# wienkers/marEx

Hardware: AMD Instinct MI355X
Metric: Mcells*timesteps/s, shifting_baseline + hobday_extreme p95 (validation+anomaly+thresholds+mask) (higher is better)
Workload: dtype f32

## Files before the change

### marex_amd/csrc/marex_tails.hip

```cpp
#include "marex_common.hip.h"
#include "marex_tails.hip.h"

typedef __amdgpu_buffer_rsrc_t tl_rsrc_t;
__device__ __forceinline__ tl_rsrc_t tl_make_rsrc(const void* base) {
    return __builtin_amdgcn_make_buffer_rsrc(const_cast<void*>(base), 0, -1, 0x00020000);
}
__device__ __forceinline__ uint4 tl_load_chunk(tl_rsrc_t r, unsigned voff, unsigned soff) {
    typedef unsigned u4 __attribute__((ext_vector_type(4)));
    const u4 v = __builtin_amdgcn_raw_buffer_load_b128(r, (int)voff, (int)soff, 0);
    return make_uint4(v.x, v.y, v.z, v.w);
}
__device__ __forceinline__ unsigned pk_sub_sat_u16(unsigned a, unsigned b) {
    unsigned r;
    asm("v_pk_sub_u16 %0, %1, %2 clamp" : "=v"(r) : "v"(a), "v"(b));
    return r;
}
__device__ __forceinline__ unsigned pk_add_u16(unsigned a, unsigned b) {
    unsigned r;
    asm("v_pk_add_u16 %0, %1, %2" : "=v"(r) : "v"(a), "v"(b));
    return r;
}
__device__ __forceinline__ unsigned pk_sub_u16(unsigned a, unsigned b) {
    unsigned r;
    asm("v_pk_sub_u16 %0, %1, %2" : "=v"(r) : "v"(a), "v"(b));
// ... 1084 lines not shown
        else if (big && p == 2 && tall)
            MAREX_TT_LAUNCH(2, 30, 1024, 34);
        else if (big && p == 2)
            MAREX_TT_LAUNCH(2, 32, 1024);
        else if (big)
            MAREX_TT_LAUNCH(3, 32, 1024);
        else if (p == 1)
            MAREX_TT_LAUNCH(1, 16, 256);
        else if (p == 2)
            MAREX_TT_LAUNCH(2, 16, 256);
        else
            MAREX_TT_LAUNCH(3, 16, 256);
    }
#undef MAREX_TT_LAUNCH
#undef MAREX_TT_ARGS
    HIP_TRY(ctx, hipGetLastError());
    return 0;
}

template <bool RING>
__global__ void __launch_bounds__(64)
k_thr_pool(const uint4* __restrict__ lists, const unsigned* __restrict__ aux, int NPER, int nch, const float* __restrict__ anom,
           long C, long c0, long c1, int nblk, const int* __restrict__ pool, int K, const float* __restrict__ centres, int nb,
           double q, int wd, float lower_bound, float upper_bound, float* __restrict__ thr, marex_thr_stats* __restrict__ stats,
           unsigned long long* __restrict__ dbg) {
    extern __shared__ uint4 pool_smem[];
    const int lane = (int)threadIdx.x;
    const long cell = c0 + (long)blockIdx.x * 64 + lane;
    const bool valid = cell < c1;
    const int d_begin = (int)blockIdx.y * NDOY / nblk, d_end = ((int)blockIdx.y + 1) * NDOY / nblk;
    const bool land = valid ? !(anom[cell] == anom[cell]) : true;
    if (__builtin_amdgcn_ballot_w64(!land) == 0) {
        if (valid)
            for (int d = d_begin; d < d_end; ++d) thr[(size_t)d * C + cell] = nan_f();
        return;
    }
    int* mem = reinterpret_cast<int*>(pool_smem) + lane;
    for (int m = 0; m < K; ++m) mem[m * 64] = land ? -1 : pool[(size_t)m * C + cell];
    uint4* ring = pool_smem + K * 16 + lane;
    const int pd = wd / 2, per_day = K * NPER, nslot = (wd * per_day + 3) & ~3;
    if (RING)
        for (int k = wd * per_day; k < nslot; ++k) ring[k * 64] = make_uint4(0, 0, 0, 0);
    const unsigned chunk_row = (unsigned)C * 16u;
    const size_t day_stride = (size_t)NPER * nch * (size_t)C;
    auto wrap = [](int d) { return d < 0 ? d + NDOY : (d >= NDOY ? d - NDOY : d); };
    auto cnt_of = [&](int day) {
        int n = 0;
        for (int m = 0; m < K; ++m) {
            const int j = mem[m * 64];
            if (j >= 0) n += (int)(aux[(size_t)day * C + j] & 0x3FFu);
        }
        return n;
    };
    auto global_first = [&](int day, int j, int p) {
        return tl_load_chunk(tl_make_rsrc(lists + (size_t)day * day_stride), (unsigned)j * 16u, (unsigned)(nch * p) * chunk_row);
    };
    auto load_day = [&](int day, int k) {
        if (!RING) return;
        for (int m = 0; m < K; ++m) {
            const int j = mem[m * 64];
            for (int p = 0; p < NPER; ++p) {
                const uint4 ch = j >= 0 ? global_first(day, j, p) : make_uint4(0, 0, 0, 0);
                ring[((k % wd) * per_day + m * NPER + p) * 64] = ch;
            }
        }
    };
    auto first_chunk = [&](int d, int i, int m, int p) {
        if (RING) return ring[(i * per_day + m * NPER + p) * 64];
        const int j = mem[m * 64];
        return j >= 0 ? global_first(wrap(d - pd + i), j, p) : make_uint4(0, 0, 0, 0);
    };
    int tot = 0;
    for (int o = 0; o < wd; ++o) {
        const int day = wrap(d_begin - pd + o);
        load_day(day, o);
        tot += cnt_of(day);
    }
    auto count_first = [&](int d, int b, int& sat) {
        const unsigned lim = ((unsigned)(b + 1) << TAIL_POS_BITS) - 1u, lim_rep = lim | (lim << 16);
        unsigned acc0 = 0, acc1 = 0, accl = 0;
        if (RING) {
            for (int k = 0; k < nslot; k += 4) {
                const uint4 c[4] = {ring[k * 64], ring[(k + 1) * 64], ring[(k + 2) * 64], ring[(k + 3) * 64]};
#pragma unroll
                for (int u = 0; u < 4; ++u) {
                    acc0 += pk_min1_u16(pk_sub_sat_u16(c[u].x, lim_rep)) + pk_min1_u16(pk_sub_sat_u16(c[u].z, lim_rep));
                    acc1 += pk_min1_u16(pk_sub_sat_u16(c[u].y, lim_rep));
                    accl += pk_min1_u16(pk_sub_sat_u16(c[u].w, lim_rep));
                }
            }
        } else
        for (int i = 0; i < wd; ++i)
            for (int m = 0; m < K; ++m)
                for (int p = 0; p < NPER; ++p) {
                    const uint4 c = first_chunk(d, i, m, p);
                    acc0 += pk_min1_u16(pk_sub_sat_u16(c.x, lim_rep)) + pk_min1_u16(pk_sub_sat_u16(c.z, lim_rep));
                    acc1 += pk_min1_u16(pk_sub_sat_u16(c.y, lim_rep));
                    accl += pk_min1_u16(pk_sub_sat_u16(c.w, lim_rep));
                }
        sat = (int)(accl >> 16);
        const unsigned acc = acc0 + acc1 + accl;
        return (int)((acc & 0xFFFFu) + (acc >> 16));
    };
    auto count_behind = [&](int d, int b, bool want) {
        const unsigned lim = ((unsigned)(b + 1) << TAIL_POS_BITS) - 1u, lim_rep = lim | (lim << 16);
        const int s0 = (d - d_begin) % wd;
        int n = 0;
        for (int i = 0; i < wd; ++i) {
            const int o = RING ? (i - s0 + wd) % wd : i;
            const tl_rsrc_t r = tl_make_rsrc(lists + (size_t)wrap(d - pd + o) * day_stride);
            for (int m = 0; m < K; ++m) {
                const int j = mem[m * 64];
                if (j < 0 || !want) continue;
                for (int p = 0; p < NPER; ++p) {
                    const uint4 c = first_chunk(d, i, m, p);
                    if ((c.w >> 16) <= lim) continue;
                    for (int jj = 1; jj < nch; ++jj) n += tl_count_above(tl_load_chunk(r, (unsigned)j * 16u, (unsigned)(nch * p + jj) * chunk_row), lim_rep);
                }
            }
        }
        return n;
    };
    unsigned kmin = 0xFFFFFFFFu, kmax = 0u, nlow = 0u, nhigh = 0u;
    unsigned long long n_exact = 0;
    for (int d = d_begin; d < d_end; ++d) {
        if (d > d_begin) {
            const int din = wrap(d + pd), dout = wrap(d - pd - 1);
            load_day(din, d - d_begin - 1);
            tot += cnt_of(din) - cnt_of(dout);
        }
        unsigned khead = 0, ktail = 0xFFFFu;
        int nlists = 0;
        auto see_head = [&](unsigned first_pair) {
            const unsigned head = first_pair & 0xFFFFu;
            khead = head > khead ? head : khead;
            ktail = (head != 0u && head < ktail) ? head : ktail;
            nlists += head != 0u ? 1 : 0;
        };
        if (RING) {
            for (int k = 0; k < nslot; k += 4) {
                const unsigned h[4] = {ring[k * 64].x, ring[(k + 1) * 64].x, ring[(k + 2) * 64].x, ring[(k + 3) * 64].x};
#pragma unroll
                for (int u = 0; u < 4; ++u) see_head(h[u]);
            }
        } else
        for (int i = 0; i < wd; ++i)
            for (int m = 0; m < K; ++m)
                for (int p = 0; p < NPER; ++p) see_head(first_chunk(d, i, m, p).x);
        float t32 = nan_f();
        if (tot > 0) {
            const double qpos = q * (double)tot;
            int lo = -1, hi = nb - 1, n_lo = tot, n_hi = 0;
            if (khead != 0u && (double)tot > qpos) {
                const int bh = (int)(khead >> TAIL_POS_BITS) - 1;
                hi = bh < hi ? bh : hi;
            }
            bool lo_exact = true;
            if (nlists > 0 && (double)(tot - nlists) <= qpos) {
                const int bt = (int)(ktail >> TAIL_POS_BITS) - 2;
                if (bt > lo && bt < hi) {
                    lo = bt;
                    n_lo = nlists;
                    lo_exact = false;
                }
            }
            while (__builtin_amdgcn_ballot_w64(hi - lo > 1) != 0) {
                const bool go = hi - lo > 1;
                const int mid = go ? (lo + hi) >> 1 : hi;
                int sat;
                int n = count_first(d, mid + 1, sat);
                bool exact = sat == 0;
                bool f = (double)(tot - n) <= qpos;
                const bool undecided = go && !f && !exact;
                if (__builtin_amdgcn_ballot_w64(undecided) != 0) {
                    const int more = count_behind(d, mid + 1, undecided);
                    if (undecided) {
                        n += more;
                        exact = true;
                        f = (double)(tot - n) <= qpos;
                        ++n_exact;
                    }
                }
                if (go) {
                    if (f) {
                        lo = mid;
                        n_lo = n;
                        lo_exact = exact;
                    } else {
                        hi = mid;
                        n_hi = n;
                    }
                }
            }
            const int iu = hi;
            const bool redo = iu > 0 && !lo_exact;
            if (__builtin_amdgcn_ballot_w64(redo) != 0) {
                int sat;
                const int ne = count_first(d, iu, sat) + count_behind(d, iu, redo);
                if (redo) {
                    n_lo = ne;
                    ++n_exact;
                }
            }
            const int il = iu > 0 ? iu - 1 : 0;
            const int cs_iu = tot - n_hi, cs_il = iu > 0 ? tot - n_lo : cs_iu;
            const int diff = cs_iu - cs_il;
            const double frac = diff > 0 ? (qpos - (double)cs_il) / (double)diff : 0.5;
            const float dc = centres[iu] - centres[il];
            const double prod = frac * (double)dc;
            t32 = (float)((double)centres[il] + prod);
            if (iu == 0) t32 = centres[0];
            if (!land) {
                const unsigned key = ordered_key(t32);
                kmin = key < kmin ? key : kmin;
                kmax = key > kmax ? key : kmax;
                if (t32 > upper_bound) ++nhigh;
                if (t32 < lower_bound) ++nlow;
            }
            if (t32 < lower_bound) t32 = lower_bound;
        }
        if (valid) thr[(size_t)d * C + cell] = land ? nan_f() : t32;
    }
    for (int sft = 32; sft > 0; sft >>= 1) {
        const unsigned a = __shfl_down(kmin, sft, 64), b = __shfl_down(kmax, sft, 64);
        kmin = a < kmin ? a : kmin;
        kmax = b > kmax ? b : kmax;
        nlow += __shfl_down(nlow, sft, 64);
        nhigh += __shfl_down(nhigh, sft, 64);
        n_exact += __shfl_down(n_exact, sft, 64);
    }
    if (lane == 0) {
        if (kmin != 0xFFFFFFFFu) atomicMin(&stats->min_key, kmin);
        if (kmax != 0u) atomicMax(&stats->max_key, kmax);
        if (nlow) atomicAdd(&stats->n_too_low, nlow);
        if (nhigh) atomicAdd(&stats->n_too_high, nhigh);
        if (dbg) {
            if (n_exact) atomicAdd(&dbg[1], n_exact);
            atomicAdd(&dbg[0], RING ? 1ull : 0ull);
            atomicAdd(&dbg[2], 1ull);
            atomicAdd(&dbg[3], (unsigned long long)(d_end - d_begin));
        }
    }
}

extern "C" int marex_hobday_thresholds_pool_f32(marex_ctx* ctx, const void* lists, const uint32_t* aux, int list_rows,
                                                const float* anom, int64_t T_out, int64_t C, int max_bucket, const int32_t* pool,
                                                int K, int64_t c0, int64_t c1, const float* centres, int nb, double q, int wd,
                                                float lower_bound, float upper_bound, float* thr_doy_major, marex_thr_stats* stats) {
    if (!ctx) return -1;
    if (!lists || !aux || !anom || !pool || !centres || !thr_doy_major || !stats || T_out <= 0 || C <= 0)
        return fail(ctx, -1, "marex_hobday_thresholds_pool_f32: null pointer or empty shape");
    if (wd < 3 || wd > 365 || (wd & 1) == 0)
        return fail(ctx, -1, "marex_hobday_thresholds_pool_f32: window_days_hobday must be odd and in 3..365");
    if (!(q > 0.0 && q <= 1.0)) return fail(ctx, -1, "marex_hobday_thresholds_pool_f32: q must be in (0, 1]");
    if (K < 1 || K > 13) return fail(ctx, -1, "marex_hobday_thresholds_pool_f32: a pool has 1..13 members (two neighbour rings), not %d", K);
    if (c0 < 0 || c0 >= c1 || c1 > C) return fail(ctx, -1, "marex_hobday_thresholds_pool_f32: need 0 <= c0 < c1 <= C");
    if (nb < 4 || nb > TAIL_MAX_NB || max_bucket < 1 || max_bucket > TAIL_MAX_BUCKET || (int64_t)max_bucket * wd * K > 65535 ||
        C > (1 << 24))
        return fail(ctx, -4, "marex_hobday_thresholds_pool_f32: shape outside the tail kernel (nb <= %d, buckets <= %d rows, "
                             "pooled window <= 65535 samples)", TAIL_MAX_NB, TAIL_MAX_BUCKET);
    HIP_TRY(ctx, hipSetDevice(ctx->device));
    int NPER, nch;
    if (!tails_geometry(max_bucket, list_rows, NPER, nch))
        return fail(ctx, -4, "marex_hobday_thresholds_pool_f32: %d rows per bucket in lists of %d", max_bucket, list_rows);
    {
        std::vector<int32_t> h((size_t)K * (size_t)C);
        HIP_TRY(ctx, hipMemcpyAsync(h.data(), pool, h.size() * sizeof(int32_t), hipMemcpyDeviceToHost, ctx->stream));
        HIP_TRY(ctx, hipStreamSynchronize(ctx->stream));
        for (int64_t c = c0; c < c1; ++c)
            if (h[(size_t)c] != (int32_t)c)
                return fail(ctx, -1, "marex_hobday_thresholds_pool_f32: row 0 of the pool table must be the cell itself (cell %lld lists %d)",
                            (long long)c, (int)h[(size_t)c]);
        for (int m = 1; m < K; ++m)
            for (int64_t c = c0; c < c1; ++c) {
                const int32_t j = h[(size_t)m * (size_t)C + (size_t)c];
                if (j < -1 || j >= C)
                    return fail(ctx, -1, "marex_hobday_thresholds_pool_f32: pool member %d of cell %lld is %d, outside -1..%lld", m,
                                (long long)c, (int)j, (long long)C - 1);
            }
    }
    const int nlist = (wd * K * NPER + 3) & ~3;
    const size_t lds_mem = (size_t)K * 64 * sizeof(int), lds_max = 128 * 1024;
    const size_t lds_ring = lds_mem + (size_t)nlist * 64 * sizeof(uint4);
    const bool use_ring = lds_ring <= lds_max && ctx_opt(ctx, "THR_POOL_RING", 1) != 0;
    const size_t lds = use_ring ? lds_ring : lds_mem;
    const long ncg = (long)((c1 - c0 + 63) / 64);
    int nblk = (int)((32L * 4 * device_cus(ctx) + ncg - 1) / ncg);
    nblk = nblk < 1 ? 1 : (nblk > 12 ? 12 : nblk);
    nblk = ctx_opt(ctx, "THR_POOL_BLOCKS", nblk);
    nblk = nblk < 1 ? 1 : (nblk > NDOY ? NDOY : nblk);
    auto kern = use_ring ? k_thr_pool<true> : k_thr_pool<false>;
    if (lds > 64 * 1024) HIP_TRY(ctx, hipFuncSetAttribute((const void*)kern, hipFuncAttributeMaxDynamicSharedMemorySize, (int)lds));
    LaunchTimer lt(ctx, MAREX_K_THRESHOLDS);
    hipLaunchKernelGGL(kern, dim3((unsigned)ncg, (unsigned)nblk), dim3(64), lds, ctx->stream, reinterpret_cast<const uint4*>(lists),
                       aux, NPER, nch, anom, (long)C, (long)c0, (long)c1, nblk, pool, K, centres, nb, q, wd, lower_bound, upper_bound,
                       thr_doy_major, stats, ctx_debug_counters(ctx));
    HIP_TRY(ctx, hipGetLastError());
    return 0;
}

#ifndef MASK_WAVES
#define MASK_WAVES 5
#endif
template <int NPERT>
__global__ void __launch_bounds__(256, MASK_WAVES)
k_mask_tails(const uint4* __restrict__ lists, const unsigned* __restrict__ aux, int NPER_all, int nch, const float* __restrict__ anom,
             const float* __restrict__ edges, int nb, const float* __restrict__ thr, const int* __restrict__ doy_start,
             const int* __restrict__ doy_rows, const long long* __restrict__ row_off, const long long* __restrict__ row_off_anom,
             long C, long c0, long c1, unsigned char* __restrict__ out, unsigned long long* __restrict__ n_true,
             unsigned long long* __restrict__ dbg) {
    const int nchunk = (int)gridDim.y;
    const int dA = (int)blockIdx.y * NDOY / nchunk, dB = ((int)blockIdx.y + 1) * NDOY / nchunk;
    const long c = (c0 & ~255L) + ((long)blockIdx.x * 256 + threadIdx.x) * 4;
    unsigned cnt_true = 0;
    unsigned long long n_slow = 0;
    if (c >= c0 && c < c1) {
        const float inv_width = (float)(nb - 1) / (edges[nb] - edges[1]);
        for (int d = dA; d < dB; ++d) {
            const int r0 = doy_start[d], nd = doy_start[d + 1] - r0;
            if (nd == 0) continue;
            const float4 th4 = *reinterpret_cast<const float4*>(thr + (size_t)d * C + c);
            const float tv[4] = {th4.x, th4.y, th4.z, th4.w};
            const uint4 ax = *reinterpret_cast<const uint4*>(aux + (size_t)d * C + c);
            const unsigned av[4] = {ax.x, ax.y, ax.z, ax.w};
            unsigned beyond = 0;
            unsigned bits[4][4];
            unsigned lim_ge[4];
            int kt[4];
            bool slow = false, walk[4];
#pragma unroll
            for (int i = 0; i < 4; ++i) {
                bits[i][0] = bits[i][1] = bits[i][2] = bits[i][3] = 0u;
                const bool isnum = tv[i] == tv[i];
                kt[i] = isnum ? digitize_bin(tv[i], edges, nb, inv_width) : nb;
                slow = slow || (isnum && (av[i] & TAIL_AUX_BEYOND) && ((av[i] & TAIL_AUX_MANY) || kt[i] >= nb));
                beyond |= (isnum && (av[i] & TAIL_AUX_BEYOND)) ? 1u : 0u;
                walk[i] = isnum && (av[i] & 0x3FFu) > 0 && kt[i] < nb;
                const unsigned lim = ((unsigned)(kt[i] + 1) << TAIL_POS_BITS) - 1u;
                lim_ge[i] = lim | (lim << 16);
            }
            auto set_prefix = [&](const uint4& q, int n, int i) {
#pragma unroll
                for (int u = 0; u < 8; ++u) {
                    const bool on = n > u;
                    if (u >= 1 && __builtin_amdgcn_ballot_w64(on) == 0) break;
                    if (on) {
                        const int pos = (int)(tl_key(q, u) & (TAIL_MAX_BUCKET - 1));
#pragma unroll
                        for (int wi = 0; wi < 4; ++wi)
                            if ((pos >> 5) == wi) bits[i][wi] |= 1u << (pos & 31);
                    }
                }
            };
            if (__builtin_amdgcn_ballot_w64(!slow) != 0)
            for (int pg = 0; pg < NPER_all; pg += NPERT) {
                const int NPER = (NPER_all - pg) < NPERT ? (NPER_all - pg) : NPERT;
                uint4 ch[NPERT][4];
                const uint4* row0 = lists + (((size_t)d * NPER_all + pg) * nch) * C + c;
#pragma unroll
                for (int p = 0; p < NPERT; ++p)
#pragma unroll
                    for (int i = 0; i < 4; ++i) ch[p][i] = p < NPER ? row0[(size_t)(p * nch) * C + i] : make_uint4(0, 0, 0, 0);
            float cand_val[NPERT][4];
            int cand_pos[NPERT][4];
            unsigned redo = 0;
            {
#pragma unroll
                for (int p = 0; p < NPERT; ++p) {
#pragma unroll
                    for (int i = 0; i < 4; ++i) {
                        cand_pos[p][i] = -1;
                        cand_val[p][i] = 0.f;
                        if (p < NPER && walk[i] && !slow) {
                            const unsigned lgt = lim_ge[i] + (0x10001u << TAIL_POS_BITS);
                            const int n_ge = tl_count_above(ch[p][i], lim_ge[i]);
                            const int n_gt = tl_count_above(ch[p][i], lgt);
                            set_prefix(ch[p][i], n_gt, i);
                            if (n_ge == 8 || n_ge - n_gt > 1) redo |= 1u << (p * 4 + i);
                            if (n_ge - n_gt == 1) {
                                const unsigned w[4] = {ch[p][i].x, ch[p][i].y, ch[p][i].z, ch[p][i].w};
                                unsigned lo = w[0], hi = w[1];
#pragma unroll
                                for (int k = 1; k < 4; ++k)
                                    if ((n_gt >> 1) == k) lo = w[k], hi = k < 3 ? w[k + 1] : 0u;
                                const unsigned key = (n_gt & 1) ? (lo >> 16) : (lo & 0xFFFFu);
                                (void)hi;
                                cand_pos[p][i] = (int)(key & (TAIL_MAX_BUCKET - 1));
                            }
                        }
                    }
                }
#pragma unroll
                for (int p = 0; p < NPERT; ++p)
#pragma unroll
                    for (int i = 0; i < 4; ++i)
                        if (cand_pos[p][i] >= 0)
                            cand_val[p][i] = *reinterpret_cast<const float*>(reinterpret_cast<const char*>(anom) + row_off_anom[r0 + cand_pos[p][i]] + (size_t)(c + i) * 4);
#pragma unroll
                for (int p = 0; p < NPERT; ++p)
#pragma unroll
                    for (int i = 0; i < 4; ++i)
                        if (cand_pos[p][i] >= 0 && cand_val[p][i] >= tv[i]) {
                            const int pos = cand_pos[p][i];
#pragma unroll
                            for (int wi = 0; wi < 4; ++wi)
                                if ((pos >> 5) == wi) bits[i][wi] |= 1u << (pos & 31);
                        }
                if (__builtin_amdgcn_ballot_w64(redo != 0u) != 0) {
#pragma unroll
                    for (int p = 0; p < NPERT; ++p)
#pragma unroll
                        for (int i = 0; i < 4; ++i) {
                            if (__builtin_amdgcn_ballot_w64((redo >> (p * 4 + i)) & 1u) == 0) continue;
                            bool on = (redo >> (p * 4 + i)) & 1u;
                            for (int jj = 0; jj < nch; ++jj) {
                                if (__builtin_amdgcn_ballot_w64(on) == 0) break;
                                const uint4 q = on ? row0[(size_t)(p * nch + jj) * C + i] : make_uint4(0, 0, 0, 0);
#pragma unroll
                                for (int u = 0; u < 8; ++u) {
                                    const unsigned key = tl_key(q, u);
                                    const int bin = (int)(key >> TAIL_POS_BITS) - 1, pos = (int)(key & (TAIL_MAX_BUCKET - 1));
                                    on = on && bin >= kt[i];
                                    if (on) {
                                        bool ext = bin > kt[i];
                                        if (!ext) ext = *reinterpret_cast<const float*>(reinterpret_cast<const char*>(anom) + row_off_anom[r0 + pos] + (size_t)(c + i) * 4) >= tv[i];
                                        if (ext) {
#pragma unroll
                                            for (int wi = 0; wi < 4; ++wi)
                                                if ((pos >> 5) == wi) bits[i][wi] |= 1u << (pos & 31);
                                        }
                                    }
                                }
                            }
                        }
                }
            }
            }
            if (__builtin_amdgcn_ballot_w64(beyond != 0u && !slow) != 0) {
#pragma unroll
                for (int i = 0; i < 4; ++i) {
                    if (!slow && tv[i] == tv[i] && (av[i] & TAIL_AUX_BEYOND)) {
                        const int p1 = (int)((av[i] >> 16) & 0x7Fu), p2 = (int)((av[i] >> 23) & 0x7Fu);
                        const bool two = (av[i] & TAIL_AUX_SECOND) != 0u;
#pragma unroll
                        for (int wi = 0; wi < 4; ++wi) {
                            if ((p1 >> 5) == wi) bits[i][wi] |= 1u << (p1 & 31);
                            if (two && (p2 >> 5) == wi) bits[i][wi] |= 1u << (p2 & 31);
                        }
                    }
                }
            }
            if (slow) {
                ++n_slow;
                for (int r = 0; r < nd; ++r) {
                    const size_t off = (size_t)doy_rows[r0 + r] * C + c;
                    const float4 a = *reinterpret_cast<const float4*>(anom + off);
                    const unsigned m0 = a.x >= tv[0], m1 = a.y >= tv[1], m2 = a.z >= tv[2], m3 = a.w >= tv[3];
                    cnt_true += m0 + m1 + m2 + m3;
                    __builtin_nontemporal_store(m0 | (m1 << 8) | (m2 << 16) | (m3 << 24), reinterpret_cast<unsigned*>(out + off));
                }
            } else {
                unsigned char* obase = out + c;
#pragma unroll
                for (int wi = 0; wi < 4; ++wi) {
                    const unsigned b0 = bits[0][wi], b1 = bits[1][wi], b2 = bits[2][wi], b3 = bits[3][wi];
                    cnt_true += __popc(b0) + __popc(b1) + __popc(b2) + __popc(b3);
                    if (wi * 32 >= nd) break;
#pragma unroll
                    for (int g = 0; g < 4; ++g) {
                        const int rlo = wi * 32 + g * 8;
                        if (rlo >= nd) break;
                        const unsigned q0 = b0 >> (g * 8), q1 = b1 >> (g * 8), q2 = b2 >> (g * 8), q3 = b3 >> (g * 8);
                        const long long* ro = row_off + r0 + rlo;
                        if (rlo + 8 <= nd) {
#pragma unroll
                            for (int rr = 0; rr < 8; ++rr) {
                                const unsigned m = ((q0 >> rr) & 1u) | (((q1 >> rr) & 1u) << 8) | (((q2 >> rr) & 1u) << 16) | (((q3 >> rr) & 1u) << 24);
                                __builtin_nontemporal_store(m, reinterpret_cast<unsigned*>(obase + ro[rr]));
                            }
                        } else {
                            for (int rr = 0; rr < nd - rlo; ++rr) {
                                const unsigned m = ((q0 >> rr) & 1u) | (((q1 >> rr) & 1u) << 8) | (((q2 >> rr) & 1u) << 16) | (((q3 >> rr) & 1u) << 24);
                                __builtin_nontemporal_store(m, reinterpret_cast<unsigned*>(obase + ro[rr]));
                            }
                        }
                    }
                }
            }
        }
    }
    if (n_true) {
        for (int s = 32; s > 0; s >>= 1) cnt_true += __shfl_down(cnt_true, s, 64);
        if ((threadIdx.x & 63) == 0 && cnt_true) atomicAdd(n_true, (unsigned long long)cnt_true);
    }
    if (dbg) {
        for (int s = 32; s > 0; s >>= 1) n_slow += __shfl_down(n_slow, s, 64);
        if ((threadIdx.x & 63) == 0 && n_slow) atomicAdd(&dbg[4], n_slow);
    }
}

extern "C" int marex_mask_ge_doy_tails_f32(marex_ctx* ctx, const void* lists, const uint32_t* aux, int list_rows, int max_bucket,
                                           const float* anom,
                                           const float* edges, int nb, const float* thr_doy_major, const int32_t* doy_start,
                                           const int32_t* doy_rows, int64_t T_out, int64_t C, int64_t c0, int64_t c1,
                                           uint8_t* extreme, unsigned long long* n_true) {
    if (!ctx) return -1;
    if (!lists || !aux || !anom || !edges || !thr_doy_major || !doy_start || !doy_rows || !extreme || T_out <= 0 || C <= 0 || nb < 4)
        return fail(ctx, -1, "marex_mask_ge_doy_tails_f32: null pointer or empty shape");
    if (c0 < 0 || c1 > C || c0 >= c1) return fail(ctx, -1, "marex_mask_ge_doy_tails_f32: need 0 <= c0 < c1 <= C");
    int NPER, nch;
    if (!tails_geometry(max_bucket, list_rows, NPER, nch))
        return fail(ctx, -4, "marex_mask_ge_doy_tails_f32: buckets must hold 1..%d rows, lists 8..32 rows", TAIL_MAX_BUCKET);
    const bool vec = (C % 4 == 0) && (c0 % 4 == 0) && (c1 % 4 == 0) && (((uintptr_t)anom | (uintptr_t)thr_doy_major) % 16 == 0) &&
                     ((uintptr_t)extreme % 4 == 0) && ((uintptr_t)aux % 16 == 0) && nb < 0x7fff;
    if (!vec)
        return marex_mask_ge_doy_f32(ctx, anom, thr_doy_major, doy_start, doy_rows, T_out, C, c0, c1, extreme, n_true);
    HIP_TRY(ctx, hipSetDevice(ctx->device));
    {
        LaunchTimer lt(ctx, MAREX_K_MASK);
        const unsigned ncb = (unsigned)(((c1 - (c0 & ~255L)) / 4 + 255) / 256);
        unsigned chunks = (16384 + ncb - 1) / ncb;
        chunks = chunks < MASK_DOY_CHUNKS ? MASK_DOY_CHUNKS : (chunks > 61 ? 61 : chunks);
        unsigned long long* dbg = ctx_debug_counters(ctx);
        const uint4* tl = reinterpret_cast<const uint4*>(lists);
        const size_t need = (size_t)T_out * sizeof(long long);
        HIP_TRY(ctx, grow_scratch(ctx->row_off_mask, ctx->row_off_mask_bytes, need));
        hipLaunchKernelGGL(k_row_offsets, dim3((unsigned)((T_out + 255) / 256)), dim3(256), 0, ctx->stream, doy_rows, (long)T_out, (long)C,
                           ctx->row_off_mask, 1);
        HIP_TRY(ctx, grow_scratch(ctx->row_off, ctx->row_off_bytes, need));
        hipLaunchKernelGGL(k_row_offsets, dim3((unsigned)((T_out + 255) / 256)), dim3(256), 0, ctx->stream, doy_rows, (long)T_out, (long)C,
                           ctx->row_off, (int)sizeof(float));
#define MAREX_MT_ARGS tl, aux, NPER, nch, anom, edges, nb, thr_doy_major, doy_start, doy_rows, ctx->row_off_mask, ctx->row_off, (long)C, (long)c0, (long)c1, extreme, n_true, dbg
        if (NPER <= 1)
            hipLaunchKernelGGL(k_mask_tails<1>, dim3(ncb, chunks), dim3(256), 0, ctx->stream, MAREX_MT_ARGS);
        else if (NPER != 3)
            hipLaunchKernelGGL(k_mask_tails<2>, dim3(ncb, chunks), dim3(256), 0, ctx->stream, MAREX_MT_ARGS);
        else
            hipLaunchKernelGGL(k_mask_tails<3>, dim3(ncb, chunks), dim3(256), 0, ctx->stream, MAREX_MT_ARGS);
#undef MAREX_MT_ARGS
    }
    HIP_TRY(ctx, hipGetLastError());
    return 0;
}
```

Before: 332,700.

## Trim register pressure in tail mask kernel with buffer loads and 32-bit offsets

Reworks k_mask_tails to cut VGPR usage. Per-lane addressing now uses 32-bit cell offsets, hidden behind an opaque asm, in place of 64-bit pointer arithmetic. List chunks are read through buffer-resource loads whose out-of-range lanes return zero without branching. The aux word is reloaded late instead of being held live, and the bitmask width NW is a template parameter so buckets of up to 96 rows keep only 3 words. Per-period unrolling is also reduced: NPERT is 1 for small buckets and 2 otherwise, dropping the 3 variant. This adds a guard that C*16 fits in 31 bits, and the smaller NPERT may reduce memory-level parallelism.

Measured after the change: 337,300, median of 6. 1.01x the previous value.

```diff
diff --git a/marex_amd/csrc/marex_tails.hip b/marex_amd/csrc/marex_tails.hip
--- a/marex_amd/csrc/marex_tails.hip
+++ b/marex_amd/csrc/marex_tails.hip
@@ -1410,7 +1410,7 @@
 #ifndef MASK_WAVES
 #define MASK_WAVES 5
 #endif
-template <int NPERT>
+template <int NPERT, int NW>
 __global__ void __launch_bounds__(256, MASK_WAVES)
 k_mask_tails(const uint4* __restrict__ lists, const unsigned* __restrict__ aux, int NPER_all, int nch, const float* __restrict__ anom,
              const float* __restrict__ edges, int nb, const float* __restrict__ thr, const int* __restrict__ doy_start,
@@ -1420,32 +1420,43 @@
     const int nchunk = (int)gridDim.y;
     const int dA = (int)blockIdx.y * NDOY / nchunk, dB = ((int)blockIdx.y + 1) * NDOY / nchunk;
     const long c = (c0 & ~255L) + ((long)blockIdx.x * 256 + threadIdx.x) * 4;
+    const unsigned cu = (unsigned)c;
+    auto cell = [&](int i) { unsigned v = cu; asm volatile("" : "+v"(v)); return v + (unsigned)i; };
+    auto lane_ptr = [](const void* base, unsigned lane_bytes) { return reinterpret_cast<const char*>(base) + lane_bytes; };
     unsigned cnt_true = 0;
-    unsigned long long n_slow = 0;
+    unsigned n_slow = 0;
     if (c >= c0 && c < c1) {
         const float inv_width = (float)(nb - 1) / (edges[nb] - edges[1]);
         for (int d = dA; d < dB; ++d) {
             const int r0 = doy_start[d], nd = doy_start[d + 1] - r0;
             if (nd == 0) continue;
-            const float4 th4 = *reinterpret_cast<const float4*>(thr + (size_t)d * C + c);
+            const float4 th4 = *reinterpret_cast<const float4*>(lane_ptr(thr + (size_t)d * C, cell(0) * 4u));
             const float tv[4] = {th4.x, th4.y, th4.z, th4.w};
-            const uint4 ax = *reinterpret_cast<const uint4*>(aux + (size_t)d * C + c);
-            const unsigned av[4] = {ax.x, ax.y, ax.z, ax.w};
             unsigned beyond = 0;
-            unsigned bits[4][4];
+            unsigned bits[4][NW];
             unsigned lim_ge[4];
-            int kt[4];
             bool slow = false, walk[4];
+            {
+                const uint4 ax = *reinterpret_cast<const uint4*>(lane_ptr(aux + (size_t)d * C, cell(0) * 4u));
+                const unsigned av[4] = {ax.x, ax.y, ax.z, ax.w};
+#pragma unroll
+                for (int i = 0; i < 4; ++i) {
+#pragma unroll
+                    for (int wi = 0; wi < NW; ++wi) bits[i][wi] = 0u;
+                    const bool isnum = tv[i] == tv[i];
+                    const int kt = isnum ? digitize_bin(tv[i], edges, nb, inv_width) : nb;
+                    slow = slow || (isnum && (av[i] & TAIL_AUX_BEYOND) && ((av[i] & TAIL_AUX_MANY) || kt >= nb));
+                    beyond |= (isnum && (av[i] & TAIL_AUX_BEYOND)) ? 1u : 0u;
+                    walk[i] = isnum && (av[i] & 0x3FFu) > 0 && kt < nb;
+                    const unsigned lim = ((unsigned)(kt + 1) << TAIL_POS_BITS) - 1u;
+                    lim_ge[i] = lim | (lim << 16);
+                }
+            }
+            unsigned voff[4];
 #pragma unroll
             for (int i = 0; i < 4; ++i) {
-                bits[i][0] = bits[i][1] = bits[i][2] = bits[i][3] = 0u;
-                const bool isnum = tv[i] == tv[i];
-                kt[i] = isnum ? digitize_bin(tv[i], edges, nb, inv_width) : nb;
-                slow = slow || (isnum && (av[i] & TAIL_AUX_BEYOND) && ((av[i] & TAIL_AUX_MANY) || kt[i] >= nb));
-                beyond |= (isnum && (av[i] & TAIL_AUX_BEYOND)) ? 1u : 0u;
-                walk[i] = isnum && (av[i] & 0x3FFu) > 0 && kt[i] < nb;
-                const unsigned lim = ((unsigned)(kt[i] + 1) << TAIL_POS_BITS) - 1u;
-                lim_ge[i] = lim | (lim << 16);
+                walk[i] = walk[i] && !slow;
+                voff[i] = walk[i] ? cell(i) * 16u : 0x80000000u;
             }
             auto set_prefix = [&](const uint4& q, int n, int i) {
 #pragma unroll
@@ -1455,7 +1466,7 @@
                     if (on) {
                         const int pos = (int)(tl_key(q, u) & (TAIL_MAX_BUCKET - 1));
 #pragma unroll
-                        for (int wi = 0; wi < 4; ++wi)
+                        for (int wi = 0; wi < NW; ++wi)
                             if ((pos >> 5) == wi) bits[i][wi] |= 1u << (pos & 31);
                     }
                 }
@@ -1464,11 +1475,14 @@
             for (int pg = 0; pg < NPER_all; pg += NPERT) {
                 const int NPER = (NPER_all - pg) < NPERT ? (NPER_all - pg) : NPERT;
                 uint4 ch[NPERT][4];
-                const uint4* row0 = lists + (((size_t)d * NPER_all + pg) * nch) * C + c;
-#pragma unroll
-                for (int p = 0; p < NPERT; ++p)
-#pragma unroll
-                    for (int i = 0; i < 4; ++i) ch[p][i] = p < NPER ? row0[(size_t)(p * nch) * C + i] : make_uint4(0, 0, 0, 0);
+                const uint4* grp = lists + (((size_t)d * NPER_all + pg) * nch) * C;
+#pragma unroll
+                for (int p = 0; p < NPERT; ++p) {
+                    const tl_rsrc_t rs = __builtin_amdgcn_make_buffer_rsrc(const_cast<uint4*>(grp + (size_t)(p * nch) * C), 0,
+                                                                           p < NPER ? (int)(C * 16) : 0, 0x00020000);
+#pragma unroll
+                    for (int i = 0; i < 4; ++i) ch[p][i] = tl_load_chunk(rs, voff[i], 0u);
+                }
             float cand_val[NPERT][4];
             int cand_pos[NPERT][4];
             unsigned redo = 0;
@@ -1479,7 +1493,7 @@
                     for (int i = 0; i < 4; ++i) {
                         cand_pos[p][i] = -1;
                         cand_val[p][i] = 0.f;
-                        if (p < NPER && walk[i] && !slow) {
+                        if (p < NPER && walk[i]) {
                             const unsigned lgt = lim_ge[i] + (0x10001u << TAIL_POS_BITS);
                             const int n_ge = tl_count_above(ch[p][i], lim_ge[i]);
                             const int n_gt = tl_count_above(ch[p][i], lgt);
@@ -1503,7 +1517,7 @@
 #pragma unroll
                     for (int i = 0; i < 4; ++i)
                         if (cand_pos[p][i] >= 0)
-                            cand_val[p][i] = *reinterpret_cast<const float*>(reinterpret_cast<const char*>(anom) + row_off_anom[r0 + cand_pos[p][i]] + (size_t)(c + i) * 4);
+                            cand_val[p][i] = *reinterpret_cast<const float*>(lane_ptr(reinterpret_cast<const char*>(anom) + row_off_anom[r0 + cand_pos[p][i]], cell(i) * 4u));
 #pragma unroll
                 for (int p = 0; p < NPERT; ++p)
 #pragma unroll
@@ -1511,7 +1525,7 @@
                         if (cand_pos[p][i] >= 0 && cand_val[p][i] >= tv[i]) {
                             const int pos = cand_pos[p][i];
 #pragma unroll
-                            for (int wi = 0; wi < 4; ++wi)
+                            for (int wi = 0; wi < NW; ++wi)
                                 if ((pos >> 5) == wi) bits[i][wi] |= 1u << (pos & 31);
                         }
                 if (__builtin_amdgcn_ballot_w64(redo != 0u) != 0) {
@@ -1521,20 +1535,21 @@
                         for (int i = 0; i < 4; ++i) {
                             if (__builtin_amdgcn_ballot_w64((redo >> (p * 4 + i)) & 1u) == 0) continue;
                             bool on = (redo >> (p * 4 + i)) & 1u;
+                            const int kt = (int)((lim_ge[i] & 0xFFFFu) >> TAIL_POS_BITS);
                             for (int jj = 0; jj < nch; ++jj) {
                                 if (__builtin_amdgcn_ballot_w64(on) == 0) break;
-                                const uint4 q = on ? row0[(size_t)(p * nch + jj) * C + i] : make_uint4(0, 0, 0, 0);
+                                const uint4 q = on ? *reinterpret_cast<const uint4*>(lane_ptr(grp + (size_t)(p * nch + jj) * C, cell(i) * 16u)) : make_uint4(0, 0, 0, 0);
 #pragma unroll
                                 for (int u = 0; u < 8; ++u) {
                                     const unsigned key = tl_key(q, u);
                                     const int bin = (int)(key >> TAIL_POS_BITS) - 1, pos = (int)(key & (TAIL_MAX_BUCKET - 1));
-                                    on = on && bin >= kt[i];
+                                    on = on && bin >= kt;
                                     if (on) {
-                                        bool ext = bin > kt[i];
-                                        if (!ext) ext = *reinterpret_cast<const float*>(reinterpret_cast<const char*>(anom) + row_off_anom[r0 + pos] + (size_t)(c + i) * 4) >= tv[i];
+                                        bool ext = bin > kt;
+                                        if (!ext) ext = *reinterpret_cast<const float*>(lane_ptr(reinterpret_cast<const char*>(anom) + row_off_anom[r0 + pos], cell(i) * 4u)) >= tv[i];
                                         if (ext) {
 #pragma unroll
-                                            for (int wi = 0; wi < 4; ++wi)
+                                            for (int wi = 0; wi < NW; ++wi)
                                                 if ((pos >> 5) == wi) bits[i][wi] |= 1u << (pos & 31);
                                         }
                                     }
@@ -1545,13 +1560,15 @@
             }
             }
             if (__builtin_amdgcn_ballot_w64(beyond != 0u && !slow) != 0) {
+                const uint4 ax = *reinterpret_cast<const uint4*>(lane_ptr(aux + (size_t)d * C, cell(0) * 4u));
+                const unsigned av[4] = {ax.x, ax.y, ax.z, ax.w};
 #pragma unroll
                 for (int i = 0; i < 4; ++i) {
                     if (!slow && tv[i] == tv[i] && (av[i] & TAIL_AUX_BEYOND)) {
                         const int p1 = (int)((av[i] >> 16) & 0x7Fu), p2 = (int)((av[i] >> 23) & 0x7Fu);
                         const bool two = (av[i] & TAIL_AUX_SECOND) != 0u;
 #pragma unroll
-                        for (int wi = 0; wi < 4; ++wi) {
+                        for (int wi = 0; wi < NW; ++wi) {
                             if ((p1 >> 5) == wi) bits[i][wi] |= 1u << (p1 & 31);
                             if (two && (p2 >> 5) == wi) bits[i][wi] |= 1u << (p2 & 31);
                         }
@@ -1561,16 +1578,15 @@
             if (slow) {
                 ++n_slow;
                 for (int r = 0; r < nd; ++r) {
-                    const size_t off = (size_t)doy_rows[r0 + r] * C + c;
-                    const float4 a = *reinterpret_cast<const float4*>(anom + off);
+                    const size_t off = (size_t)doy_rows[r0 + r] * C;
+                    const float4 a = *reinterpret_cast<const float4*>(lane_ptr(anom + off, cell(0) * 4u));
                     const unsigned m0 = a.x >= tv[0], m1 = a.y >= tv[1], m2 = a.z >= tv[2], m3 = a.w >= tv[3];
                     cnt_true += m0 + m1 + m2 + m3;
-                    __builtin_nontemporal_store(m0 | (m1 << 8) | (m2 << 16) | (m3 << 24), reinterpret_cast<unsigned*>(out + off));
+                    __builtin_nontemporal_store(m0 | (m1 << 8) | (m2 << 16) | (m3 << 24), reinterpret_cast<unsigned*>(out + off + cell(0)));
                 }
             } else {
-                unsigned char* obase = out + c;
-#pragma unroll
-                for (int wi = 0; wi < 4; ++wi) {
+#pragma unroll
+                for (int wi = 0; wi < NW; ++wi) {
                     const unsigned b0 = bits[0][wi], b1 = bits[1][wi], b2 = bits[2][wi], b3 = bits[3][wi];
                     cnt_true += __popc(b0) + __popc(b1) + __popc(b2) + __popc(b3);
                     if (wi * 32 >= nd) break;
@@ -1584,12 +1600,12 @@
 #pragma unroll
                             for (int rr = 0; rr < 8; ++rr) {
                                 const unsigned m = ((q0 >> rr) & 1u) | (((q1 >> rr) & 1u) << 8) | (((q2 >> rr) & 1u) << 16) | (((q3 >> rr) & 1u) << 24);
-                                __builtin_nontemporal_store(m, reinterpret_cast<unsigned*>(obase + ro[rr]));
+                                __builtin_nontemporal_store(m, reinterpret_cast<unsigned*>(out + ro[rr] + cu));
                             }
                         } else {
                             for (int rr = 0; rr < nd - rlo; ++rr) {
                                 const unsigned m = ((q0 >> rr) & 1u) | (((q1 >> rr) & 1u) << 8) | (((q2 >> rr) & 1u) << 16) | (((q3 >> rr) & 1u) << 24);
-                                __builtin_nontemporal_store(m, reinterpret_cast<unsigned*>(obase + ro[rr]));
+                                __builtin_nontemporal_store(m, reinterpret_cast<unsigned*>(out + ro[rr] + cu));
                             }
                         }
                     }
@@ -1603,7 +1619,7 @@
     }
     if (dbg) {
         for (int s = 32; s > 0; s >>= 1) n_slow += __shfl_down(n_slow, s, 64);
-        if ((threadIdx.x & 63) == 0 && n_slow) atomicAdd(&dbg[4], n_slow);
+        if ((threadIdx.x & 63) == 0 && n_slow) atomicAdd(&dbg[4], (unsigned long long)n_slow);
     }
 }
 
@@ -1620,7 +1636,8 @@
     if (!tails_geometry(max_bucket, list_rows, NPER, nch))
         return fail(ctx, -4, "marex_mask_ge_doy_tails_f32: buckets must hold 1..%d rows, lists 8..32 rows", TAIL_MAX_BUCKET);
     const bool vec = (C % 4 == 0) && (c0 % 4 == 0) && (c1 % 4 == 0) && (((uintptr_t)anom | (uintptr_t)thr_doy_major) % 16 == 0) &&
-                     ((uintptr_t)extreme % 4 == 0) && ((uintptr_t)aux % 16 == 0) && nb < 0x7fff;
+                     ((uintptr_t)extreme % 4 == 0) && ((uintptr_t)aux % 16 == 0) && nb < 0x7fff &&
+                     C * 16 < 0x80000000ll;
     if (!vec)
         return marex_mask_ge_doy_f32(ctx, anom, thr_doy_major, doy_start, doy_rows, T_out, C, c0, c1, extreme, n_true);
     HIP_TRY(ctx, hipSetDevice(ctx->device));
@@ -1639,12 +1656,10 @@
         hipLaunchKernelGGL(k_row_offsets, dim3((unsigned)((T_out + 255) / 256)), dim3(256), 0, ctx->stream, doy_rows, (long)T_out, (long)C,
                            ctx->row_off, (int)sizeof(float));
 #define MAREX_MT_ARGS tl, aux, NPER, nch, anom, edges, nb, thr_doy_major, doy_start, doy_rows, ctx->row_off_mask, ctx->row_off, (long)C, (long)c0, (long)c1, extreme, n_true, dbg
-        if (NPER <= 1)
-            hipLaunchKernelGGL(k_mask_tails<1>, dim3(ncb, chunks), dim3(256), 0, ctx->stream, MAREX_MT_ARGS);
-        else if (NPER != 3)
-            hipLaunchKernelGGL(k_mask_tails<2>, dim3(ncb, chunks), dim3(256), 0, ctx->stream, MAREX_MT_ARGS);
+        if (max_bucket <= 96)
+            hipLaunchKernelGGL((k_mask_tails<1, 3>), dim3(ncb, chunks), dim3(256), 0, ctx->stream, MAREX_MT_ARGS);
         else
-            hipLaunchKernelGGL(k_mask_tails<3>, dim3(ncb, chunks), dim3(256), 0, ctx->stream, MAREX_MT_ARGS);
+            hipLaunchKernelGGL((k_mask_tails<2, 4>), dim3(ncb, chunks), dim3(256), 0, ctx->stream, MAREX_MT_ARGS);
 #undef MAREX_MT_ARGS
     }
     HIP_TRY(ctx, hipGetLastError());
```
